# zichunhao/lgn-autoencoder

Hardware: AMD Instinct MI355X
Metric: jets/sec fwd+bwd, 30-particle maxdim=2 bs=512 (higher is better)
Workload: dtype f64

## Files before the change

### lgn-autoencoder_amd/csrc/api.hip

```cpp
#include "net.hpp"

using namespace lgn;

extern "C" {

int lgn_level_fwd_f64(int B, int N, int C, int CO, int decoder, const double* s_in, const double* v_in, const double* p,
                      const uint8_t* mask, const double* ra, const double* rb, const double* rc, const double* w0,
                      const double* b0, const double* w1, const double* b1, const double* wm0, const double* wm1,
                      double* ag0, double* ag1, double* s_out, double* v_out, void* stream) {
  LGN_CHECK_ARG(s_in && v_in && p && b0 && b1 && wm0 && wm1 && ag0 && ag1 && s_out && v_out, "level_fwd: null pointer");
  LGN_CHECK_ARG(decoder || (mask && ra && rb && rc && w0 && w1), "level_fwd: encoder needs mask and radial parameters");
  LevelArgs<double> a{B, N, C, CO, s_in, v_in, p, mask, ra, rb, rc, w0, b0, w1, b1, wm0, wm1, ag0, ag1, s_out, v_out};
  a.flags = level_flags_from_env();
  return level_fwd_dispatch<double>(a, decoder, (hipStream_t)stream);
}

int lgn_level_bwd_partial_rows(int B, int N, int decoder, int* rows_mix, int* rows_rad) {
  LGN_CHECK_ARG(B > 0 && N > 0 && rows_mix && rows_rad, "level_bwd_partial_rows: bad arguments");
  level_bwd_partial_rows(B, N, decoder, level_flags_from_env(), rows_mix, rows_rad);
  return 0;
}

int lgn_level_rad_partial_len(int C, int decoder) { return rad_partial_size(C, decoder != 0); }
int lgn_level_jet_split(int B, int N) { return N <= 40 ? level_jet_split(B, N) : 1; }

int lgn_level_bwd_f64(int B, int N, int C, int CO, int decoder, const double* s_in, const double* v_in, const double* p,
                      const uint8_t* mask, const double* ra, const double* rb, const double* rc, const double* w0,
                      const double* b0, const double* w1, const double* b1, const double* wm0, const double* wm1,
                      const double* ag0, const double* ag1, const double* g_s_out, const double* g_v_out, double* g_ag,
                      double* g_s_in, double* g_v_in, double* g_p, double* part_mix, double* part_rad, void* stream) {
  LGN_CHECK_ARG(s_in && v_in && p && b0 && b1 && wm0 && wm1 && ag0 && ag1 && g_s_out && g_v_out && g_ag && g_s_in &&
                    g_v_in && part_mix && part_rad, "level_bwd: null pointer");
  LGN_CHECK_ARG(decoder ? (g_p != nullptr) : (mask && ra && rb && rc && w0 && w1), "level_bwd: missing decoder g_p / encoder radial parameters");
  LevelBwdArgs<double> a{B, N, C, CO, s_in, v_in, p, mask, ra, rb, rc, w0, b0, w1, b1, wm0, wm1, ag0, ag1,
                         g_s_out, g_v_out, g_ag, g_s_in, g_v_in, g_p, part_mix, part_rad};
  a.flags = level_flags_from_env();
  return level_bwd_dispatch<double>(a, decoder, (hipStream_t)stream);
}

int lgn_cg_product_fwd_f64(int R, int N, int C, int D1, int D2, int DO, int mode, int nnz, const int* row_ptr, const int* col,
                           const double* coef, const double* x1, const double* x2, double* out, void* stream) {
  return cg_product_fwd(R, N, C, D1, D2, DO, mode, nnz, row_ptr, col, coef, x1, x2, out, (hipStream_t)stream);
}
int lgn_cg_product_bwd_f64(int R, int N, int C, int D1, int D2, int DO, int mode, int nnz, const int* row_ptr, const int* col,
                           const double* coef, const double* x1, const double* x2, const double* g_out, double* g_x1, double* g_x2,
                           void* stream) {
  return cg_product_bwd(R, N, C, D1, D2, DO, mode, nnz, row_ptr, col, coef, x1, x2, g_out, g_x1, g_x2, (hipStream_t)stream);
}

int lgn_reduce_partials_f64(const double* part, int rows, int n, double* out, int accumulate, void* stream) {
  LGN_CHECK_ARG(part && out && rows > 0 && n >= 0, "reduce_partials: bad arguments");
// ... 172 lines not shown
```

### lgn-autoencoder_amd/csrc/level_bwd.hip

```cpp
#include <stdlib.h>

#include "level_dev.hpp"
#include <type_traits>
#include "ops.hpp"
#include "tail_dev.hpp"

namespace lgn {

template <int C> struct GA {
  static constexpr int A3 = 0, A4 = 2 * C, A1 = 4 * C, A2 = 12 * C, SIZE = 20 * C;
};

template <typename T, int C>
__global__ __launch_bounds__(BLOCK) void level_bwd_mix_kernel(LevelBwdArgs<T> a) {
  constexpr int IT = 32;
  constexpr int K = 5 * C;
  constexpr int XS = K * 10;
  const int N = a.N, B = a.B, CO = a.CO;
  const int b = blockIdx.x, tile = blockIdx.y, tid = threadIdx.x;
  const int GS = CO * 10;

  extern __shared__ __align__(16) unsigned char smem_raw[];
  T* sm = reinterpret_cast<T*>(smem_raw);
  T* wm = sm;
// ... 338 lines not shown
    }
  }
  return 0;
}

int level_bwd_nodes2_dispatch(const LevelBwdArgs<double>& a, int decoder, hipStream_t stream);
int level_bwd_rad2_dispatch(const LevelBwdArgs<double>& a, hipStream_t stream);

int level_bwd3_dispatch(const LevelBwdArgs<double>& a, int decoder, hipStream_t stream);
int level_bwd_dec_sep_dispatch(const LevelBwdArgs<double>& a, hipStream_t stream);
int level_bwd_sweep_enc_dispatch(const LevelBwdArgs<double>& a, hipStream_t stream);
static bool dec_pairwise(int flags) { return (flags & LVL_DEC_PAIRWISE) != 0; }
bool level_bwd3_fits(int N);

static bool use_v3(int N, int flags) { return !(flags & LVL_LEVEL_V2) && level_bwd3_fits(N); }

bool level_bwd_carries_input(int N, int flags) { return use_v3(N, flags); }

void level_bwd_partial_rows(int B, int N, int decoder, int flags, int* rows_mix, int* rows_rad) {
  const int tiles = cdiv(N, 32);
  if (use_v3(N, flags)) {
    const int split = (decoder && !dec_pairwise(flags)) ? 1 : level_jet_split(B, N);
    *rows_mix = B * split;
    *rows_rad = B * split;
    return;
  }
  *rows_mix = B * tiles;
  if (decoder && dec_pairwise(flags)) {
    *rows_rad = B * tiles;
  } else {
// ... 135 lines not shown
```

### lgn-autoencoder_amd/csrc/level_bwd3.hip

```cpp
#include "level_dev.hpp"
#include "ops.hpp"
#include "wave_sum.hpp"

namespace lgn {

typedef double v4d __attribute__((ext_vector_type(4)));

namespace {
__device__ __forceinline__ double dppq(double v, int xor2) {
  int lo = __double2loint(v), hi = __double2hiint(v);
  if (xor2) {
    lo = __builtin_amdgcn_mov_dpp(lo, 0x4E, 0xF, 0xF, true);
    hi = __builtin_amdgcn_mov_dpp(hi, 0x4E, 0xF, 0xF, true);
  } else {
    lo = __builtin_amdgcn_mov_dpp(lo, 0xB1, 0xF, 0xF, true);
    hi = __builtin_amdgcn_mov_dpp(hi, 0xB1, 0xF, 0xF, true);
  }
  return __hiloint2double(hi, lo);
}
__device__ __forceinline__ double quad_sum(double v) {
  v += dppq(v, 0);
  v += dppq(v, 1);
  return v;
}
// ... 34 lines not shown
  static constexpr int SMS = 52;
  static constexpr int SEPSZ = DEC ? SMS * C : 0;
  static size_t smem(int N, int CO) {
    return sizeof(double) * ((((size_t)N * NS + 1) & ~size_t(1)) + (size_t)N * (20 * C + 2) + (size_t)N * 10 * C + (size_t)N * PS +
                             scratch(N, CO) + SEPSZ) + N + 16;
  }
};

template <int C, bool DEC, bool SEP, int NWV, bool SYM = false>
__global__ __launch_bounds__(64 * NWV) __attribute__((amdgpu_waves_per_eu(C <= 4 || DEC ? 2 : 1, C <= 4 || DEC ? 2 : 1))) void level_bwd3_kernel(LevelBwdArgs<double> a) {
  static_assert(!SYM || !DEC, "the symmetric sweep is the encoder's");
  using F = Bwd3<C, DEC, NWV>;
  constexpr int BLK = F::BLK;
  using G = GA3<C>;
  constexpr int NG = F::NG, NS = F::NS, PS = F::PS, K = 5 * C;
  const int N = a.N, B = a.B, CO = a.CO;
  const int b = blockIdx.x, tid = threadIdx.x, lane = tid & 63, wave = tid >> 6;
  const int ngroups = (N + 3) >> 2, gper = (ngroups + (int)gridDim.y - 1) / (int)gridDim.y;
  const int glo = min(ngroups, (int)blockIdx.y * gper), ghi = min(ngroups, glo + gper);
  const int nlo = min(N, 4 * glo), nhi = min(N, 4 * ghi);
  const size_t prow = (size_t)b * gridDim.y + blockIdx.y;

  extern __shared__ __align__(16) unsigned char smem_raw[];
  double* nd = reinterpret_cast<double*>(smem_raw);
  double* ga = nd + ((N * NS + 1) & ~1);
  double* gd = ga + N * G::SIZE;
  double* pj = gd + N * 10 * C;
  double* tr = pj + N * PS;
  double* go = tr;
  double* wm = go + N * 10 * CO;
  double* agl = wm + 4 * CO * K;
  double* sm = tr + F::scratch(N, CO);
  uint8_t* mk = reinterpret_cast<uint8_t*>(sm + F::SEPSZ);

  STAMP(0);
  {
    const size_t plo = (size_t)B * N * CO, pa = (size_t)B * N * 2 * C;
    JetRegs<double> jr;
    load_jet_issue<double, C, DEC>(a.s_in, a.v_in, a.p, a.mask, B, N, b, jr);
    const int eg = tid < N * CO ? tid : 0, ea_ = tid < N * 2 * C ? tid : 0, ew = tid < 2 * CO * K ? tid : 0;
    const size_t ig = (size_t)b * N * CO + eg, ia = (size_t)b * N * 2 * C + ea_;
    double rg[10], ra[10];
    rg[0] = a.g_s_out[ig];
    rg[1] = a.g_s_out[plo + ig];
    ra[0] = a.ag0[ia];
    ra[1] = a.ag0[pa + ia];
#pragma unroll
    for (int m = 0; m < 4; ++m) {
      rg[2 + m] = a.g_v_out[ig * 4 + m];
      rg[6 + m] = a.g_v_out[plo * 4 + ig * 4 + m];
      ra[2 + m] = a.ag1[ia * 4 + m];
      ra[6 + m] = a.ag1[(pa + ia) * 4 + m];
    }
    const double w0v = a.wm0[ew], w1v = a.wm1[ew];
    load_jet_commit<double, C, DEC>(a.s_in, a.v_in, a.p, a.mask, B, N, b, jr, nd, pj, mk);
    if (tid < N * CO) {
#pragma unroll
      for (int m = 0; m < 10; ++m) go[tid * 10 + m] = rg[m];
    }
    if (tid < N * 2 * C) {
#pragma unroll
      for (int m = 0; m < 10; ++m) agl[tid * 10 + m] = ra[m];
    }
    if (tid < 2 * CO * K) {
      wm[tid] = w0v;
      wm[2 * CO * K + tid] = w1v;
    }
    for (int e = tid + BLK; e < 2 * CO * K; e += BLK) {
      wm[e] = a.wm0[e];
      wm[2 * CO * K + e] = a.wm1[e];
    }
    for (int e = tid + BLK; e < N * CO; e += BLK) {
      const size_t idx = (size_t)b * N * CO + e;
      double* g = go + e * 10;
      g[0] = a.g_s_out[idx];
      g[1] = a.g_s_out[plo + idx];
#pragma unroll
      for (int m = 0; m < 4; ++m) {
        g[2 + m] = a.g_v_out[idx * 4 + m];
        g[6 + m] = a.g_v_out[plo * 4 + idx * 4 + m];
      }
    }
    for (int e = tid + BLK; e < N * 2 * C; e += BLK) {
      const size_t ea = (size_t)b * N * 2 * C + e;
      double* x = agl + e * 10;
      x[0] = a.ag0[ea];
      x[1] = a.ag0[pa + ea];
#pragma unroll
      for (int m = 0; m < 4; ++m) {
        x[2 + m] = a.ag1[ea * 4 + m];
        x[6 + m] = a.ag1[(pa + ea) * 4 + m];
      }
    }
  }
  __syncthreads();
  STAMP(1);

  {
    const int half = tid >= BLK / 2;
    for (int e = half ? tid - BLK / 2 : tid; e < N * C; e += BLK / 2) {
      const int n = e / C, c = e - n * C;
      const double* w0r = wm + c;
      const double* w1r = wm + 2 * CO * K + c;
      if (half == 0) {
        cx<double> gx0[2] = {{0, 0}, {0, 0}}, gx1[2][4] = {{{0, 0}, {0, 0}, {0, 0}, {0, 0}}, {{0, 0}, {0, 0}, {0, 0}, {0, 0}}};
        for (int o = 0; o < CO; ++o) {
          const double* g = go + (n * CO + o) * 10;
          const cx<double> gs = {g[0], g[1]};
          cx<double> gv[4];
#pragma unroll
          for (int m = 0; m < 4; ++m) gv[m] = {g[2 + m], g[6 + m]};
// ... 48 lines not shown
#pragma unroll
        for (int m = 0; m < 4; ++m) {
          cfmac(gs, b34[m], v[m]);
          cx<double> gv = b2[m];
          cfmac(gv, b34[m], s);
          cfmac(gv, a3, vt[m]);
          gdn[2 + m] = gv.r;
          gdn[6 + m] = gv.i;
        }
        gdn[0] = gs.r;
        gdn[1] = gs.i;
      }
    }
  }
  STAMP(2);
  {
    double* part = a.part_mix + prow * (4 * CO * K);
    constexpr int NPART = F::MIXP;
    const int OK = CO * K, nper = (nhi - nlo + NPART - 1) / NPART;
    const int pi = tid / K, k = tid - pi * K;
    cx<double> d0[8], d1[8];
#pragma unroll
    for (int o = 0; o < 8; ++o) d0[o] = d1[o] = {0, 0};
    if (pi < NPART) {
      const int q = k / C, c = k - q * C;
      const int n1 = min(nhi, nlo + (pi + 1) * nper);
      for (int n = nlo + pi * nper; n < n1; ++n) {
        cx<double> x0, x1[4];
        if (q < 2) {
          const double* x = agl + (n * 2 * C + k) * 10;
          x0 = {x[0], x[1]};
#pragma unroll
          for (int m = 0; m < 4; ++m) x1[m] = {x[2 + m], x[6 + m]};
        } else {
          const double* ni = nd + n * NS + c * 10;
          const cx<double> s = {ni[0], ni[1]};
          cx<double> v[4];
#pragma unroll
          for (int m = 0; m < 4; ++m) v[m] = {ni[2 + m], ni[6 + m]};
          if (q == 2) {
            x0 = s;
#pragma unroll
            for (int m = 0; m < 4; ++m) x1[m] = v[m];
          } else {
            if (q == 3) { x0 = bil2(v, v); x0.r *= 0.5; x0.i *= 0.5; } else x0 = cmul(s, s);
#pragma unroll
            for (int m = 0; m < 4; ++m) x1[m] = cmul(v[m], s);
          }
// ... 22 lines not shown
    }
    STAMP(50);
    __syncthreads();
    STAMP(51);
    for (int ex = tid; ex < 4 * OK; ex += BLK) {
      const int e = ex >> 2, x = ex & 3;
      double v = red[ex];
#pragma unroll
      for (int pp = 1; pp < NPART; ++pp) v += red[pp * OK * 4 + ex];
      part[x * OK + e] = v;
    }
  }

  if constexpr (DEC && SEP) {
    STAMP(3);
    __syncthreads();
    STAMP(4);
    if (tid < 64) {
      const int k = tid & 7, part = tid >> 3;
      double mean = 0.0;
      for (int n = part; n < N; n += 8) mean += pj[n * 8 + k];
      mean += shfl_xor(mean, 8);
      mean += shfl_xor(mean, 16);
      mean += shfl_xor(mean, 32);
      if (part == 0) sm[k] = mean / N;
    }
    __syncthreads();
    for (int e = tid; e < N * 8; e += BLK) pj[e] -= sm[e & 7];
    __syncthreads();
#define LGN_PUT(k, val)                                       \
  do {                                                        \
    if ((k) < 16) a0[(k) < 16 ? (k) : 0] += (val);                                        \
    else if ((k) < 32) a1[(k) >= 16 && (k) < 32 ? (k) - 16 : 0] += (val);                 \
    else if ((k) < 44) a2[(k) >= 32 && (k) < 44 ? (k) - 32 : 0] += (val);                 \
    else a3[(k) >= 44 ? (k) - 44 : 0] += (val);                                           \
  } while (0)
    for (int c = wave; c < C; c += NWV) {
      double a0[16], a1[16], a2[12], a3[8];
#pragma unroll
      for (int k = 0; k < 16; ++k) a0[k] = a1[k] = 0.0;
#pragma unroll
      for (int k = 0; k < 12; ++k) a2[k] = 0.0;
#pragma unroll
      for (int k = 0; k < 8; ++k) a3[k] = 0.0;
      for (int n = lane; n < N; n += 64) {
        const double* ni = nd + n * NS + c * 10;
        const double* pn = pj + n * 8;
        const double* gi = ga + n * G::SIZE;
        cx<double> pc[4], v[4];
#pragma unroll
        for (int m = 0; m < 4; ++m) {
          pc[m] = {pn[m], pn[4 + m]};
          v[m] = {ni[2 + m], ni[6 + m]};
        }
        const cx<double> sn = {ni[0], ni[1]};
        LGN_PUT(0, sn.r);  LGN_PUT(1, sn.i);
#pragma unroll
        for (int m = 0; m < 4; ++m) {
          LGN_PUT(2 + 2 * m, v[m].r);  LGN_PUT(3 + 2 * m, v[m].i);
          const cx<double> sp = cmul(sn, pc[m]);
          LGN_PUT(10 + 2 * m, sp.r);  LGN_PUT(11 + 2 * m, sp.i);
        }
        const cx<double> vp = bil2(v, pc);
        LGN_PUT(18, vp.r);  LGN_PUT(19, vp.i);
        const cx<double> g3 = {0.5 * gi[G::A3 + 2 * c], 0.5 * gi[G::A3 + 2 * c + 1]};
        LGN_PUT(20, gi[G::A4 + 2 * c]);  LGN_PUT(21, gi[G::A4 + 2 * c + 1]);
        LGN_PUT(22, g3.r);  LGN_PUT(23, g3.i);
        cx<double> gp2 = {0, 0};
#pragma unroll
        for (int m = 0; m < 4; ++m) {
          const cx<double> g1 = {gi[G::A1 + (c * 4 + m) * 2], gi[G::A1 + (c * 4 + m) * 2 + 1]};
          const cx<double> g2 = {gi[G::A2 + (c * 4 + m) * 2], gi[G::A2 + (c * 4 + m) * 2 + 1]};
          LGN_PUT(24 + 2 * m, g1.r);  LGN_PUT(25 + 2 * m, g1.i);
          LGN_PUT(32 + 2 * m, g2.r);  LGN_PUT(33 + 2 * m, g2.i);
          cfmac(gp2, g2, pc[m]);
          const cx<double> gp3 = cmulc(g3, pc[m]);
          LGN_PUT(42 + 2 * m, gp3.r);  LGN_PUT(43 + 2 * m, gp3.i);
        }
        LGN_PUT(40, gp2.r);  LGN_PUT(41, gp2.i);
      }
      double* q = sm + c * F::SMS;
      wave_sum_store<16>(a0, q, lane);
      wave_sum_store<16>(a1, q + 16, lane);
      wave_sum_store<12>(a2, q + 32, lane);
      wave_sum_store<8>(a3, q + 44, lane);
    }
#undef LGN_PUT
    __syncthreads();

    STAMP(5);
    const size_t pls = (size_t)B * N * C;
    for (int e = tid; e < N * C; e += BLK) {
      const int n = e / C, c = e - n * C;
      const double* q = sm + c * F::SMS;
      const double* pn = pj + n * 8;
      const double* gdn = gd + e * 10;
      const cx<double> R0 = {a.b0[c], a.b0[c]}, R1 = {a.b1[c], a.b1[c]};
      const cx<double> e0 = {R0.r - R0.i, R0.r + R0.i};
      cx<double> pc[4], pt[4];
#pragma unroll
// ... 633 lines not shown
```

### lgn-autoencoder_amd/csrc/level_dev.hpp

```cpp
#pragma once
#include "level.hpp"

namespace lgn {

template <int C, bool DEC>
struct Carve {
  static constexpr int R = 4 * C;
  static constexpr int NS = node_stride(C);
  static constexpr int PS = DEC ? 8 : 4;
  static constexpr int RA = 0, RB = NB, RC = 2 * NB;
  static constexpr int RW = 3 * NB;
  static constexpr int RBIAS = RW + NB * R;
  static constexpr int RAD_SIZE = RBIAS + R;
  __host__ __device__ static constexpr int even(int x) { return (x + 1) & ~1; }
};

template <typename T>
struct JetRegs {
  T s[2], v[8], p[2];
  uint8_t m;
};
template <typename T, int C, bool DEC>
__device__ __forceinline__ void load_jet_issue(const T* __restrict__ s_in, const T* __restrict__ v_in, const T* __restrict__ p,
                                               const uint8_t* __restrict__ mask, int B, int N, int b, JetRegs<T>& r) {
// ... 160 lines not shown
  cx<T> t = cmul(a[2], b[2]);
  r.r -= t.r;
  r.i -= t.i;
  cfma(r, a[3], b[1]);
  return r;
}

template <typename T>
__device__ __forceinline__ void metric_perm(const cx<T> (&x)[4], cx<T> (&y)[4]) {
  y[0] = x[0];
  y[1] = x[3];
  y[2] = {-x[2].r, -x[2].i};
  y[3] = x[1];
}

__device__ __forceinline__ void rcp5(const double (&u)[5], double (&r)[5]) {
  const double p1 = u[0] * u[1], p2 = p1 * u[2], p3 = p2 * u[3], p4 = p3 * u[4];
  if (__builtin_expect(!(p4 < 0x1p+1000), 0)) {
#pragma unroll
    for (int s = 0; s < 5; ++s) r[s] = 1.0 / u[s];
    return;
  }
  double t = __builtin_amdgcn_rcp(p4);
  double e = __builtin_fma(-p4, t, 1.0);
  t = __builtin_fma(t, e, t);
  e = __builtin_fma(-p4, t, 1.0);
  t = __builtin_fma(t, e, t);
  r[4] = t * p3;  t *= u[4];
  r[3] = t * p2;  t *= u[3];
  r[2] = t * p1;  t *= u[2];
// ... 6 lines not shown
```

### lgn-autoencoder_amd/csrc/level_fwd2.hip

```cpp
#include "level_dev.hpp"
#include "net_dev.hpp"
#include "ops.hpp"
#include "wave_sum.hpp"

namespace lgn {

typedef double v4d __attribute__((ext_vector_type(4)));
LGN_STAMP_DECL
LGN_STAMP_READER(lgn_debug_stamps_fwd2)

__device__ __forceinline__ double dpp_quad(double v, int ctrl_is_xor2) {
  int lo = __double2loint(v), hi = __double2hiint(v);
  if (ctrl_is_xor2) {
    lo = __builtin_amdgcn_mov_dpp(lo, 0x4E, 0xF, 0xF, true);
    hi = __builtin_amdgcn_mov_dpp(hi, 0x4E, 0xF, 0xF, true);
  } else {
    lo = __builtin_amdgcn_mov_dpp(lo, 0xB1, 0xF, 0xF, true);
    hi = __builtin_amdgcn_mov_dpp(hi, 0xB1, 0xF, 0xF, true);
  }
  return __hiloint2double(hi, lo);
}
__device__ __forceinline__ double quad_sum(double v) {
  v += dpp_quad(v, 0);
  v += dpp_quad(v, 1);
// ... 118 lines not shown
    }
  }
#pragma unroll
  for (int g = 0; g < NG; ++g) {
    const int ch = 4 * g + cg;
#pragma unroll
    for (int q = 0; q < 4; ++q) {
      const double* bb = (q >> 1) ? a.b1 : a.b0;
      bias[g][q] = ch < C ? (DEC ? bb[ch] : bb[2 * ch + (q & 1)]) : 0.0;
    }
  }
  __syncthreads();
  STAMP(1);

  if constexpr (DEC && SEP) {
    if (tid < 64) {
      const int k = tid & 7, part = tid >> 3;
      double mean = 0.0;
      for (int n = part; n < N; n += 8) mean += pj[n * 8 + k];
      mean += shfl_xor(mean, 8);
      mean += shfl_xor(mean, 16);
      mean += shfl_xor(mean, 32);
      if (part == 0) sums[k] = mean / N;
    }
    __syncthreads();
    for (int e = tid; e < N * 8; e += nthr) pj[e] -= sums[e & 7];
    __syncthreads();
#define LGN_PUT(k, val)                                           \
  do {                                                            \
    if ((k) < 12) a0[(k) < 12 ? (k) : 0] += (val);                \
    else a1[(k) >= 12 ? (k) - 12 : 0] += (val);                   \
  } while (0)
    for (int c = wave; c < C; c += nw) {
      double a0[12], a1[8];
#pragma unroll
      for (int k = 0; k < 12; ++k) a0[k] = 0.0;
#pragma unroll
      for (int k = 0; k < 8; ++k) a1[k] = 0.0;
      for (int n = lane; n < N; n += 64) {
        const double* ni = nd + n * F::NS + c * 10;
        const double* pn = pj + n * 8;
        const cx<double> sn = {ni[0], ni[1]};
        cx<double> v[4], pc[4];
#pragma unroll
        for (int m = 0; m < 4; ++m) {
          v[m] = {ni[2 + m], ni[6 + m]};
          pc[m] = {pn[m], pn[4 + m]};
        }
        LGN_PUT(0, sn.r);  LGN_PUT(1, sn.i);
#pragma unroll
        for (int m = 0; m < 4; ++m) {
          LGN_PUT(2 + 2 * m, v[m].r);  LGN_PUT(3 + 2 * m, v[m].i);
          const cx<double> sp = cmul(sn, pc[m]);
          LGN_PUT(10 + 2 * m, sp.r);  LGN_PUT(11 + 2 * m, sp.i);
        }
        const cx<double> vp = bil2(v, pc);
        LGN_PUT(18, vp.r);  LGN_PUT(19, vp.i);
      }
      wave_sum_store<12>(a0, sums + c * 20, lane);
      wave_sum_store<8>(a1, sums + c * 20 + 12, lane);
    }
#undef LGN_PUT
    __syncthreads();
  }

  const int ngroups = (N + 3) >> 2, gper = (ngroups + (int)gridDim.y - 1) / (int)gridDim.y;
  const int rlo = min(N, 4 * (int)blockIdx.y * gper), rhi = min(N, rlo + 4 * gper);
  auto catmix = [&](int c0, int c1) {
    constexpr int K = 5 * C;
    const int nr = c1 - c0;
    const size_t plo = (size_t)B * N * CO;
    if (wave == 0) {
      for (int rl = lane; rl < nr; rl += 64) {
        const int r = c0 + rl;
        const double* st = agl + rl * F::AGS;
        const double* ni = nd + r * F::NS;
        cx<double> x[K];
// ... 45 lines not shown
          cx<double> acc = {0, 0};
#pragma unroll
          for (int k = 0; k < K; ++k) cfma(acc, cx<double>{wr[k], wi[k]}, x[k]);
          const size_t e = ((size_t)b * N + r) * CO + o;
          a.v_out[e * 4 + m] = acc.r;
          a.v_out[plo * 4 + e * 4 + m] = acc.i;
        }
      }
    }
    };
  for (int c0 = rlo; c0 < rhi; c0 += chunk) {
  const int c1 = min(rhi, c0 + chunk);
  if constexpr (DEC && SEP) {
    for (int e = tid; e < (c1 - c0) * C; e += nthr) {
      const int rl = e / C, c = e - rl * C, n = c0 + rl;
      const double* sm = sums + c * 20;
      const double* pn = pj + n * 8;
      const cx<double> R0 = {a.b0[c], a.b0[c]}, R1 = {a.b1[c], a.b1[c]};
      const cx<double> e0 = {R0.r - R0.i, R0.r + R0.i};
      const cx<double> S = {sm[0], sm[1]};
      cx<double> VS[4], pc[4];
#pragma unroll
      for (int m = 0; m < 4; ++m) {
        VS[m] = {sm[2 + 2 * m], sm[3 + 2 * m]};
        pc[m] = {pn[m], pn[4 + m]};
      }
      double* st = agl + rl * F::AGS;
      const cx<double> a4 = cmul(S, e0);
      cx<double> t = bil2(VS, pc);
      t.r -= sm[18];  t.i -= sm[19];
      cx<double> a3 = cmul(R1, t);
      st[F::A3 + 2 * c] = 0.5 * a3.r;  st[F::A3 + 2 * c + 1] = 0.5 * a3.i;
      st[F::A4 + 2 * c] = a4.r;        st[F::A4 + 2 * c + 1] = a4.i;
#pragma unroll
      for (int m = 0; m < 4; ++m) {
        const cx<double> a1 = cmul(VS[m], e0);
        cx<double> u = cmul(pc[m], S);
        u.r -= sm[10 + 2 * m];  u.i -= sm[11 + 2 * m];
        const cx<double> a2 = cmul(R1, u);
        st[F::A1 + (c * 4 + m) * 2] = a1.r;  st[F::A1 + (c * 4 + m) * 2 + 1] = a1.i;
        st[F::A2 + (c * 4 + m) * 2] = a2.r;  st[F::A2 + (c * 4 + m) * 2 + 1] = a2.i;
      }
    }
  } else {
  const int ngr = (c1 - c0 + 3) >> 2;
  const int rs = (!DEC && nw == 4 && ngr >= 1 && ngr <= 2 && chunk >= 16) ? 4 / ngr : 1;
  const int rpart = rs > 1 ? wave % rs : 0, ntl = (N + 3) >> 2;
  auto row_group = [&](const int rg, const int jlo, const int jhi, const int slab) __attribute__((always_inline)) {
    const int i0 = rg * 4;
    const int i = i0 + ti;
    const bool iok = i < N;
    const int ii = iok ? i : N - 1;
    double pi[F::PS];
#pragma unroll
    for (int m = 0; m < F::PS; ++m) pi[m] = pj[ii * F::PS + m];
    const bool mi = DEC ? false : (mk[ii] != 0);
// ... 147 lines not shown
    for (int rg = (c0 >> 2) + wave; rg * 4 < c1; rg += nw) row_group(rg, 0, N, 0);
  }
  if (rs > 1) {
    __syncthreads();
    const int tot = 4 * ngr * F::AGS;
    for (int e = tid; e < tot; e += nthr) {
      double v = agl[e];
      for (int pp = 1; pp < rs; ++pp) v += agl[pp * tot + e];
      agl[e] = v;
    }
  }
  }
  __syncthreads();
  STAMP(20);

  if constexpr (TRAIN) {
    const size_t pl0 = (size_t)B * N * 2 * C;
    for (int e = tid; e < (c1 - c0) * 2 * C; e += nthr) {
      const int n = e / (2 * C), r = e - n * 2 * C, blk = r / C, ch = r - blk * C;
      const double* st = agl + n * F::AGS + (blk ? F::A4 : F::A3) + 2 * ch;
      const size_t ge = ((size_t)b * N + c0) * 2 * C + e;
      a.ag0[ge] = st[0];
      a.ag0[pl0 + ge] = st[1];
    }
    for (int e = tid; e < (c1 - c0) * 2 * C * 4; e += nthr) {
      const int n = e / (8 * C), r = e - n * 8 * C, blk = r / (4 * C), cm = r - blk * 4 * C;
      const double* st = agl + n * F::AGS + (blk ? F::A2 : F::A1) + 2 * cm;
      const size_t ge = ((size_t)b * N + c0) * 8 * C + e;
      a.ag1[ge] = st[0];
      a.ag1[pl0 * 4 + ge] = st[1];
    }
// ... 38 lines not shown
  auto kern = level_fwd2_kernel<C, DEC, SEP, TRAIN>;
  if (smem > 64 * 1024) {
    hipError_t e = hipFuncSetAttribute(reinterpret_cast<const void*>(kern), hipFuncAttributeMaxDynamicSharedMemorySize, (int)smem);
    if (e != hipSuccess) { set_error("hipFuncSetAttribute: %s", hipGetErrorString(e)); return (int)e; }
  }
  const int nthreads = wide ? 2 * BLOCK : BLOCK;
  const int split = (SEP || a.N > 40) ? 1 : level_jet_split(a.B, a.N);
  hipLaunchKernelGGL(kern, dim3(a.B, split), dim3(nthreads), smem, stream, a, chunk);
  LGN_CHECK_LAUNCH();
  return 0;
}

bool level_fwd_carries_loss(int N, int flags) { return N <= 40 && !(flags & LVL_DEC_PAIRWISE); }

template <bool TRAIN>
static int level_fwd_run(const LevelArgs<double>& a, int decoder, hipStream_t stream) {
  LGN_CHECK_ARG(a.B > 0 && a.N > 0, "level_fwd: empty batch (B=%d N=%d)", a.B, a.N);
  LGN_CHECK_ARG(!a.in_w0 || (!decoder && a.in_w1 && a.in_s && a.in_v), "level_fwd: the input stage rides on encoder levels only");
  LGN_CHECK_ARG(a.CO >= 1 && a.CO <= 8, "level_fwd: C_out=%d unsupported (1..8)", a.CO);
  const bool pairwise = (a.flags & LVL_DEC_PAIRWISE) != 0;
#define LGN_CASE(CC)                                                                                         \
  case CC:                                                                                                   \
    if (!decoder) return launch_level_fwd2<CC, false, false, TRAIN>(a, stream);                              \
    return pairwise ? launch_level_fwd2<CC, true, false, TRAIN>(a, stream) : launch_level_fwd2<CC, true, true, TRAIN>(a, stream);
  switch (a.C) {
#ifdef LGN_DEV_ONLY_C4
    LGN_CASE(4)
#else
    LGN_CASE(1) LGN_CASE(2) LGN_CASE(3) LGN_CASE(4) LGN_CASE(5) LGN_CASE(6) LGN_CASE(7) LGN_CASE(8)
#endif
    default:
// ... 15 lines not shown
```

### lgn-autoencoder_amd/csrc/ops.hpp

```cpp
#pragma once
#include <cstdlib>
#include <vector>
#include "level.hpp"

namespace lgn {

template <typename T> int level_fwd_dispatch(const LevelArgs<T>&, int decoder, hipStream_t);
int level_fwd_eval(const LevelArgs<double>&, int decoder, hipStream_t);
template <typename T> int level_bwd_dispatch(const LevelBwdArgs<T>&, int decoder, hipStream_t);
template <typename T> int reduce_partials(const T* part, int rows, int n, T* out, int accumulate, hipStream_t);
template <typename T> int reduce_partials_strided(const T* part, int rows, int stride, int col0, int n, T* out, hipStream_t);
constexpr int RED_MAX_SEG = 64;
template <typename T> struct RedSeg { const T* part; int rows, stride, col0, n; T* out; };
template <typename T> struct RedJob {
  int nseg;
  RedSeg<T> seg[RED_MAX_SEG];
  int tile0[RED_MAX_SEG + 1];
  void add(const T* part, int rows, int stride, int col0, int n, T* out) { seg[nseg++] = RedSeg<T>{part, rows, stride, col0, n, out}; }
};
template <typename T> int reduce_segments(RedJob<T>& job, hipStream_t);
template <typename T>
int rad_finalize(const T* tot, int C, const T* ra, const T* rb, const T* rc, const T* w0, const T* w1, T* g_a, T* g_b, T* g_c,
                 T* g_w0, T* g_b0, T* g_w1, T* g_b1, hipStream_t);
struct RadFinJob {
// ... 7 lines not shown
  double *m, *v;
  long* step_dev;
  double lambda, lr, beta1, beta2, eps;
  int do_adam;
  const double* loss_part;
  int nB;
  double* loss_out;
  int reduce_only;
  unsigned long long* counters;
  int opt_form = 0;
  int kind = 0;
  double l2 = 0.0, alpha = 0.0, mu = 0.0;
};
int step_tail(const std::vector<RedSeg<double>>& segs, const RadFinJob& fin, const StepTailArgs& ta, hipStream_t st);
void level_bwd_partial_rows(int B, int N, int decoder, int flags, int* rows_mix, int* rows_rad);
bool level_bwd_carries_input(int N, int flags);
bool level_fwd_carries_loss(int N, int flags);

constexpr int MLP_MAX_LIN = 8;
template <typename T>
struct MlpArgs {
  int M;
  int C;
  int H;
  int nlin;
  const T* w[MLP_MAX_LIN];
  const T* b[MLP_MAX_LIN];
  const T* s_in;
  T* s_out;
  const T* g_out;
// ... 127 lines not shown
```

### lgn-autoencoder_amd/csrc/step.hip

```cpp
#include <stdlib.h>

#include <algorithm>
#include <mutex>
#include <vector>

#include "net.hpp"
#include "../../include/lgn_amd.h"

namespace lgn {
namespace {

struct Bump {
  double* base;
  size_t off = 0;
  double* take(size_t n) {
    n = (n + 15) & ~size_t(15);
    double* p = base ? base + off : nullptr;
    off += n;
    return p;
  }
};

struct NetBuf {
  double *s[5], *v[5], *smix[4], *ag0[4], *ag1[4];
// ... 139 lines not shown
  Work w{};
  Bump b{base};
  const int Nd = dec_nodes(d), Nmax = d.N > Nd ? d.N : Nd;
  const size_t BNe = (size_t)d.B * d.N, BNd = (size_t)d.B * Nd, BN = (size_t)d.B * Nmax;
  const int L = d.n_levels;
  int cmax = 0;
  for (int l = 0; l <= L; ++l) cmax = cmax > d.enc_channels[l] ? cmax : d.enc_channels[l], cmax = cmax > d.dec_channels[l] ? cmax : d.dec_channels[l];
  auto net = [&](NetBuf& n, const int* ch, bool dec) {
    const size_t BN = dec ? BNd : BNe;
    for (int l = 0; l <= L; ++l) {
      n.s[l] = b.take(2 * BN * ch[l]);
      n.v[l] = b.take(8 * BN * ch[l]);
    }
    for (int l = 0; l < L; ++l) {
      n.smix[l] = b.take(2 * BN * ch[l + 1]);
      n.ag0[l] = b.take(4 * BN * ch[l]);
      n.ag1[l] = b.take(16 * BN * ch[l]);
      const size_t hs = l + 1 < L && BN <= mlp_save_max_rows()
                            ? mlp_saved_doubles((int)BN, d.mlp_hidden_mul * 2 * ch[l + 1], d.mlp_nlin) : 0;
      n.hsave[l] = hs ? b.take(hs) : nullptr;
    }
  };
  net(w.enc, d.enc_channels, false);
  net(w.dec, d.dec_channels, true);
  const int Ts = d.tau_s, Tv = d.tau_v, PB = pool_blocks(d.latent_pool);
  w.lat_s = b.take((size_t)2 * d.B * PB * Ts);
  w.lat_v = b.take((size_t)2 * d.B * PB * Tv * 4);
  w.g_lat_v = b.take((size_t)2 * d.B * PB * Tv * 4);
  w.pdec = b.take(8 * BN);
  for (int q = 0; q < 2; ++q) {
    w.gs[q] = b.take(2 * BN * cmax);
    w.gv[q] = b.take(8 * BN * cmax);
// ... 708 lines not shown
  double* pdec;
  int* idx;
  size_t total;
};
NetAct carve_act(const lgn_net_desc& d, bool dec, double* base) {
  NetAct a{};
  Bump b{base};
  const size_t BN = (size_t)d.B * d.N;
  const int* ch = dec ? d.dec_channels : d.enc_channels;
  for (int l = 0; l <= d.n_levels; ++l) {
    a.n.s[l] = b.take(2 * BN * ch[l]);
    a.n.v[l] = b.take(8 * BN * ch[l]);
  }
  for (int l = 0; l < d.n_levels; ++l) {
    a.n.smix[l] = b.take(2 * BN * ch[l + 1]);
    a.n.ag0[l] = b.take(4 * BN * ch[l]);
    a.n.ag1[l] = b.take(16 * BN * ch[l]);
    const size_t hs = BN <= mlp_save_max_rows()
                          ? mlp_saved_doubles((int)BN, d.mlp_hidden_mul * 2 * ch[l + 1], d.mlp_nlin) : 0;
    a.n.hsave[l] = hs ? b.take(hs) : nullptr;
  }
  if (dec) a.pdec = b.take(8 * BN);
  else a.idx = reinterpret_cast<int*>(b.take(((size_t)d.B * 2 * (d.tau_s + d.tau_v) * 2 + 1) / 2 + 8));
  a.total = b.off;
  return a;
}

struct NetScratch {
  Work w;
  size_t total;
};
NetScratch carve_scratch(const lgn_net_desc& d, bool dec, double* base) {
// ... 591 lines not shown
```

Measured before the change: 1.067 million.

## Recompute decoder separable aggregates in backward instead of storing them

For the decoder's separable (non-pairwise) path under the v3 backward, the forward no longer writes the per-node aggregate tensors ag0/ag1, and no workspace is allocated for them. The backward kernel instead rebuilds them: it recentres the momenta, computes per-channel jet sums into shared memory, and evaluates the aggregate on the fly in the mix-gradient loop. The shared helper code is factored out of the forward kernel. This removes global writes and reads of the aggregates and shrinks the workspace, at the cost of extra arithmetic, an extra barrier and shared-memory reductions in the backward.

```diff
diff --git a/lgn-autoencoder_amd/csrc/api.hip b/lgn-autoencoder_amd/csrc/api.hip
--- a/lgn-autoencoder_amd/csrc/api.hip
+++ b/lgn-autoencoder_amd/csrc/api.hip
@@ -8,10 +8,12 @@
                       const uint8_t* mask, const double* ra, const double* rb, const double* rc, const double* w0,
                       const double* b0, const double* w1, const double* b1, const double* wm0, const double* wm1,
                       double* ag0, double* ag1, double* s_out, double* v_out, void* stream) {
-  LGN_CHECK_ARG(s_in && v_in && p && b0 && b1 && wm0 && wm1 && ag0 && ag1 && s_out && v_out, "level_fwd: null pointer");
+  const int flags = level_flags_from_env();
+  LGN_CHECK_ARG(s_in && v_in && p && b0 && b1 && wm0 && wm1 && s_out && v_out && ((ag0 && ag1) || !level_saves_aggregate(N, decoder, flags)),
+                "level_fwd: null pointer");
   LGN_CHECK_ARG(decoder || (mask && ra && rb && rc && w0 && w1), "level_fwd: encoder needs mask and radial parameters");
   LevelArgs<double> a{B, N, C, CO, s_in, v_in, p, mask, ra, rb, rc, w0, b0, w1, b1, wm0, wm1, ag0, ag1, s_out, v_out};
-  a.flags = level_flags_from_env();
+  a.flags = flags;
   return level_fwd_dispatch<double>(a, decoder, (hipStream_t)stream);
 }
 
@@ -29,12 +31,13 @@
                       const double* b0, const double* w1, const double* b1, const double* wm0, const double* wm1,
                       const double* ag0, const double* ag1, const double* g_s_out, const double* g_v_out, double* g_ag,
                       double* g_s_in, double* g_v_in, double* g_p, double* part_mix, double* part_rad, void* stream) {
-  LGN_CHECK_ARG(s_in && v_in && p && b0 && b1 && wm0 && wm1 && ag0 && ag1 && g_s_out && g_v_out && g_ag && g_s_in &&
-                    g_v_in && part_mix && part_rad, "level_bwd: null pointer");
+  const int flags = level_flags_from_env();
+  LGN_CHECK_ARG(s_in && v_in && p && b0 && b1 && wm0 && wm1 && g_s_out && g_v_out && g_ag && g_s_in && g_v_in && part_mix && part_rad &&
+                    ((ag0 && ag1) || !level_saves_aggregate(N, decoder, flags)), "level_bwd: null pointer");
   LGN_CHECK_ARG(decoder ? (g_p != nullptr) : (mask && ra && rb && rc && w0 && w1), "level_bwd: missing decoder g_p / encoder radial parameters");
   LevelBwdArgs<double> a{B, N, C, CO, s_in, v_in, p, mask, ra, rb, rc, w0, b0, w1, b1, wm0, wm1, ag0, ag1,
                          g_s_out, g_v_out, g_ag, g_s_in, g_v_in, g_p, part_mix, part_rad};
-  a.flags = level_flags_from_env();
+  a.flags = flags;
   return level_bwd_dispatch<double>(a, decoder, (hipStream_t)stream);
 }
 
diff --git a/lgn-autoencoder_amd/csrc/level_bwd.hip b/lgn-autoencoder_amd/csrc/level_bwd.hip
--- a/lgn-autoencoder_amd/csrc/level_bwd.hip
+++ b/lgn-autoencoder_amd/csrc/level_bwd.hip
@@ -376,6 +376,8 @@
 bool level_bwd3_fits(int N);
 
 static bool use_v3(int N, int flags) { return !(flags & LVL_LEVEL_V2) && level_bwd3_fits(N); }
+
+bool level_saves_aggregate(int N, int decoder, int flags) { return !(decoder && !dec_pairwise(flags) && use_v3(N, flags)); }
 
 bool level_bwd_carries_input(int N, int flags) { return use_v3(N, flags); }
 
diff --git a/lgn-autoencoder_amd/csrc/level_bwd3.hip b/lgn-autoencoder_amd/csrc/level_bwd3.hip
--- a/lgn-autoencoder_amd/csrc/level_bwd3.hip
+++ b/lgn-autoencoder_amd/csrc/level_bwd3.hip
@@ -72,6 +72,7 @@
   constexpr int BLK = F::BLK;
   using G = GA3<C>;
   constexpr int NG = F::NG, NS = F::NS, PS = F::PS, K = 5 * C;
+  constexpr bool REBUILD = DEC && SEP;
   const int N = a.N, B = a.B, CO = a.CO;
   const int b = blockIdx.x, tid = threadIdx.x, lane = tid & 63, wave = tid >> 6;
   const int ngroups = (N + 3) >> 2, gper = (ngroups + (int)gridDim.y - 1) / (int)gridDim.y;
@@ -101,14 +102,19 @@
     double rg[10], ra[10];
     rg[0] = a.g_s_out[ig];
     rg[1] = a.g_s_out[plo + ig];
-    ra[0] = a.ag0[ia];
-    ra[1] = a.ag0[pa + ia];
 #pragma unroll
     for (int m = 0; m < 4; ++m) {
       rg[2 + m] = a.g_v_out[ig * 4 + m];
       rg[6 + m] = a.g_v_out[plo * 4 + ig * 4 + m];
-      ra[2 + m] = a.ag1[ia * 4 + m];
-      ra[6 + m] = a.ag1[(pa + ia) * 4 + m];
+    }
+    if constexpr (!REBUILD) {
+      ra[0] = a.ag0[ia];
+      ra[1] = a.ag0[pa + ia];
+#pragma unroll
+      for (int m = 0; m < 4; ++m) {
+        ra[2 + m] = a.ag1[ia * 4 + m];
+        ra[6 + m] = a.ag1[(pa + ia) * 4 + m];
+      }
     }
     const double w0v = a.wm0[ew], w1v = a.wm1[ew];
     load_jet_commit<double, C, DEC>(a.s_in, a.v_in, a.p, a.mask, B, N, b, jr, nd, pj, mk);
@@ -116,9 +122,11 @@
 #pragma unroll
       for (int m = 0; m < 10; ++m) go[tid * 10 + m] = rg[m];
     }
-    if (tid < N * 2 * C) {
-#pragma unroll
-      for (int m = 0; m < 10; ++m) agl[tid * 10 + m] = ra[m];
+    if constexpr (!REBUILD) {
+      if (tid < N * 2 * C) {
+#pragma unroll
+        for (int m = 0; m < 10; ++m) agl[tid * 10 + m] = ra[m];
+      }
     }
     if (tid < 2 * CO * K) {
       wm[tid] = w0v;
@@ -139,20 +147,26 @@
         g[6 + m] = a.g_v_out[plo * 4 + idx * 4 + m];
       }
     }
-    for (int e = tid + BLK; e < N * 2 * C; e += BLK) {
-      const size_t ea = (size_t)b * N * 2 * C + e;
-      double* x = agl + e * 10;
-      x[0] = a.ag0[ea];
-      x[1] = a.ag0[pa + ea];
-#pragma unroll
-      for (int m = 0; m < 4; ++m) {
-        x[2 + m] = a.ag1[ea * 4 + m];
-        x[6 + m] = a.ag1[(pa + ea) * 4 + m];
+    if constexpr (!REBUILD) {
+      for (int e = tid + BLK; e < N * 2 * C; e += BLK) {
+        const size_t ea = (size_t)b * N * 2 * C + e;
+        double* x = agl + e * 10;
+        x[0] = a.ag0[ea];
+        x[1] = a.ag0[pa + ea];
+#pragma unroll
+        for (int m = 0; m < 4; ++m) {
+          x[2 + m] = a.ag1[ea * 4 + m];
+          x[6 + m] = a.ag1[(pa + ea) * 4 + m];
+        }
       }
     }
   }
   __syncthreads();
   STAMP(1);
+  if constexpr (REBUILD) {
+    sep_centre_momenta(pj, N, sm);
+    for (int c = wave; c < C; c += NWV) sep_jet_sums<NS>(nd, pj, N, c, lane, sm + c * F::SMS);
+  }
 
   {
     const int half = tid >= BLK / 2;
@@ -231,6 +245,7 @@
     }
   }
   STAMP(2);
+  if constexpr (REBUILD) __syncthreads();
   {
     double* part = a.part_mix + prow * (4 * CO * K);
     constexpr int NPART = F::MIXP;
@@ -242,13 +257,23 @@
     if (pi < NPART) {
       const int q = k / C, c = k - q * C;
       const int n1 = min(nhi, nlo + (pi + 1) * nper);
+      double b0c = 0.0, b1c = 0.0;
+      if constexpr (REBUILD) { b0c = a.b0[c]; b1c = a.b1[c]; }
       for (int n = nlo + pi * nper; n < n1; ++n) {
         cx<double> x0, x1[4];
         if (q < 2) {
-          const double* x = agl + (n * 2 * C + k) * 10;
-          x0 = {x[0], x[1]};
-#pragma unroll
-          for (int m = 0; m < 4; ++m) x1[m] = {x[2 + m], x[6 + m]};
+          if constexpr (REBUILD) {
+            cx<double> a3, a4, a1[4], a2[4];
+            sep_aggregate(sm + c * F::SMS, pj + n * 8, b0c, b1c, a3, a4, a1, a2);
+            x0 = q == 0 ? a3 : a4;
+#pragma unroll
+            for (int m = 0; m < 4; ++m) x1[m] = q == 0 ? a1[m] : a2[m];
+          } else {
+            const double* x = agl + (n * 2 * C + k) * 10;
+            x0 = {x[0], x[1]};
+#pragma unroll
+            for (int m = 0; m < 4; ++m) x1[m] = {x[2 + m], x[6 + m]};
+          }
         } else {
           const double* ni = nd + n * NS + c * 10;
           const cx<double> s = {ni[0], ni[1]};
@@ -301,55 +326,22 @@
 
   if constexpr (DEC && SEP) {
     STAMP(3);
-    __syncthreads();
     STAMP(4);
-    if (tid < 64) {
-      const int k = tid & 7, part = tid >> 3;
-      double mean = 0.0;
-      for (int n = part; n < N; n += 8) mean += pj[n * 8 + k];
-      mean += shfl_xor(mean, 8);
-      mean += shfl_xor(mean, 16);
-      mean += shfl_xor(mean, 32);
-      if (part == 0) sm[k] = mean / N;
-    }
-    __syncthreads();
-    for (int e = tid; e < N * 8; e += BLK) pj[e] -= sm[e & 7];
-    __syncthreads();
 #define LGN_PUT(k, val)                                       \
   do {                                                        \
-    if ((k) < 16) a0[(k) < 16 ? (k) : 0] += (val);                                        \
-    else if ((k) < 32) a1[(k) >= 16 && (k) < 32 ? (k) - 16 : 0] += (val);                 \
-    else if ((k) < 44) a2[(k) >= 32 && (k) < 44 ? (k) - 32 : 0] += (val);                 \
-    else a3[(k) >= 44 ? (k) - 44 : 0] += (val);                                           \
+    if ((k) < 36) a1[(k) >= 20 && (k) < 36 ? (k) - 20 : 0] += (val);                      \
+    else a2[(k) >= 36 ? (k) - 36 : 0] += (val);                                           \
   } while (0)
     for (int c = wave; c < C; c += NWV) {
-      double a0[16], a1[16], a2[12], a3[8];
-#pragma unroll
-      for (int k = 0; k < 16; ++k) a0[k] = a1[k] = 0.0;
-#pragma unroll
-      for (int k = 0; k < 12; ++k) a2[k] = 0.0;
-#pragma unroll
-      for (int k = 0; k < 8; ++k) a3[k] = 0.0;
+      double a1[16], a2[16];
+#pragma unroll
+      for (int k = 0; k < 16; ++k) a1[k] = a2[k] = 0.0;
       for (int n = lane; n < N; n += 64) {
-        const double* ni = nd + n * NS + c * 10;
         const double* pn = pj + n * 8;
         const double* gi = ga + n * G::SIZE;
-        cx<double> pc[4], v[4];
-#pragma unroll
-        for (int m = 0; m < 4; ++m) {
-          pc[m] = {pn[m], pn[4 + m]};
-          v[m] = {ni[2 + m], ni[6 + m]};
-        }
-        const cx<double> sn = {ni[0], ni[1]};
-        LGN_PUT(0, sn.r);  LGN_PUT(1, sn.i);
-#pragma unroll
-        for (int m = 0; m < 4; ++m) {
-          LGN_PUT(2 + 2 * m, v[m].r);  LGN_PUT(3 + 2 * m, v[m].i);
-          const cx<double> sp = cmul(sn, pc[m]);
-          LGN_PUT(10 + 2 * m, sp.r);  LGN_PUT(11 + 2 * m, sp.i);
-        }
-        const cx<double> vp = bil2(v, pc);
-        LGN_PUT(18, vp.r);  LGN_PUT(19, vp.i);
+        cx<double> pc[4];
+#pragma unroll
+        for (int m = 0; m < 4; ++m) pc[m] = {pn[m], pn[4 + m]};
         const cx<double> g3 = {0.5 * gi[G::A3 + 2 * c], 0.5 * gi[G::A3 + 2 * c + 1]};
         LGN_PUT(20, gi[G::A4 + 2 * c]);  LGN_PUT(21, gi[G::A4 + 2 * c + 1]);
         LGN_PUT(22, g3.r);  LGN_PUT(23, g3.i);
@@ -367,10 +359,8 @@
         LGN_PUT(40, gp2.r);  LGN_PUT(41, gp2.i);
       }
       double* q = sm + c * F::SMS;
-      wave_sum_store<16>(a0, q, lane);
-      wave_sum_store<16>(a1, q + 16, lane);
-      wave_sum_store<12>(a2, q + 32, lane);
-      wave_sum_store<8>(a3, q + 44, lane);
+      wave_sum_store<16>(a1, q + 20, lane);
+      wave_sum_store<16>(a2, q + 36, lane);
     }
 #undef LGN_PUT
     __syncthreads();
diff --git a/lgn-autoencoder_amd/csrc/level_dev.hpp b/lgn-autoencoder_amd/csrc/level_dev.hpp
--- a/lgn-autoencoder_amd/csrc/level_dev.hpp
+++ b/lgn-autoencoder_amd/csrc/level_dev.hpp
@@ -1,5 +1,6 @@
 #pragma once
 #include "level.hpp"
+#include "wave_sum.hpp"
 
 namespace lgn {
 
@@ -198,6 +199,84 @@
   y[3] = x[1];
 }
 
+__device__ __forceinline__ void sep_centre_momenta(double* pj, int N, double* mean8) {
+  const int tid = threadIdx.x, nthr = blockDim.x;
+  if (tid < 64) {
+    const int k = tid & 7, part = tid >> 3;
+    double mean = 0.0;
+    for (int n = part; n < N; n += 8) mean += pj[n * 8 + k];
+    mean += shfl_xor(mean, 8);
+    mean += shfl_xor(mean, 16);
+    mean += shfl_xor(mean, 32);
+    if (part == 0) mean8[k] = mean / N;
+  }
+  __syncthreads();
+  for (int e = tid; e < N * 8; e += nthr) pj[e] -= mean8[e & 7];
+  __syncthreads();
+}
+
+template <int NS>
+__device__ __forceinline__ void sep_jet_sums(const double* nd, const double* pj, int N, int c, int lane, double* dst) {
+#define LGN_PUT(k, val)                                           \
+  do {                                                            \
+    if ((k) < 12) a0[(k) < 12 ? (k) : 0] += (val);                \
+    else a1[(k) >= 12 ? (k) - 12 : 0] += (val);                   \
+  } while (0)
+  double a0[12], a1[8];
+#pragma unroll
+  for (int k = 0; k < 12; ++k) a0[k] = 0.0;
+#pragma unroll
+  for (int k = 0; k < 8; ++k) a1[k] = 0.0;
+  for (int n = lane; n < N; n += 64) {
+    const double* ni = nd + n * NS + c * 10;
+    const double* pn = pj + n * 8;
+    const cx<double> sn = {ni[0], ni[1]};
+    cx<double> v[4], pc[4];
+#pragma unroll
+    for (int m = 0; m < 4; ++m) {
+      v[m] = {ni[2 + m], ni[6 + m]};
+      pc[m] = {pn[m], pn[4 + m]};
+    }
+    LGN_PUT(0, sn.r);  LGN_PUT(1, sn.i);
+#pragma unroll
+    for (int m = 0; m < 4; ++m) {
+      LGN_PUT(2 + 2 * m, v[m].r);  LGN_PUT(3 + 2 * m, v[m].i);
+      const cx<double> sp = cmul(sn, pc[m]);
+      LGN_PUT(10 + 2 * m, sp.r);  LGN_PUT(11 + 2 * m, sp.i);
+    }
+    const cx<double> vp = bil2(v, pc);
+    LGN_PUT(18, vp.r);  LGN_PUT(19, vp.i);
+  }
+  wave_sum_store<12>(a0, dst, lane);
+  wave_sum_store<8>(a1, dst + 12, lane);
+#undef LGN_PUT
+}
+
+__device__ __forceinline__ void sep_aggregate(const double* sm, const double* pn, double b0c, double b1c, cx<double>& a3,
+                                              cx<double>& a4, cx<double> (&a1)[4], cx<double> (&a2)[4]) {
+  const cx<double> R0 = {b0c, b0c}, R1 = {b1c, b1c};
+  const cx<double> e0 = {R0.r - R0.i, R0.r + R0.i};
+  const cx<double> S = {sm[0], sm[1]};
+  cx<double> VS[4], pc[4];
+#pragma unroll
+  for (int m = 0; m < 4; ++m) {
+    VS[m] = {sm[2 + 2 * m], sm[3 + 2 * m]};
+    pc[m] = {pn[m], pn[4 + m]};
+  }
+  a4 = cmul(S, e0);
+  cx<double> t = bil2(VS, pc);
+  t.r -= sm[18];  t.i -= sm[19];
+  const cx<double> r3 = cmul(R1, t);
+  a3 = {0.5 * r3.r, 0.5 * r3.i};
+#pragma unroll
+  for (int m = 0; m < 4; ++m) {
+    a1[m] = cmul(VS[m], e0);
+    cx<double> u = cmul(pc[m], S);
+    u.r -= sm[10 + 2 * m];  u.i -= sm[11 + 2 * m];
+    a2[m] = cmul(R1, u);
+  }
+}
+
 __device__ __forceinline__ void rcp5(const double (&u)[5], double (&r)[5]) {
   const double p1 = u[0] * u[1], p2 = p1 * u[2], p3 = p2 * u[3], p4 = p3 * u[4];
   if (__builtin_expect(!(p4 < 0x1p+1000), 0)) {
diff --git a/lgn-autoencoder_amd/csrc/level_fwd2.hip b/lgn-autoencoder_amd/csrc/level_fwd2.hip
--- a/lgn-autoencoder_amd/csrc/level_fwd2.hip
+++ b/lgn-autoencoder_amd/csrc/level_fwd2.hip
@@ -156,53 +156,8 @@
   STAMP(1);
 
   if constexpr (DEC && SEP) {
-    if (tid < 64) {
-      const int k = tid & 7, part = tid >> 3;
-      double mean = 0.0;
-      for (int n = part; n < N; n += 8) mean += pj[n * 8 + k];
-      mean += shfl_xor(mean, 8);
-      mean += shfl_xor(mean, 16);
-      mean += shfl_xor(mean, 32);
-      if (part == 0) sums[k] = mean / N;
-    }
-    __syncthreads();
-    for (int e = tid; e < N * 8; e += nthr) pj[e] -= sums[e & 7];
-    __syncthreads();
-#define LGN_PUT(k, val)                                           \
-  do {                                                            \
-    if ((k) < 12) a0[(k) < 12 ? (k) : 0] += (val);                \
-    else a1[(k) >= 12 ? (k) - 12 : 0] += (val);                   \
-  } while (0)
-    for (int c = wave; c < C; c += nw) {
-      double a0[12], a1[8];
-#pragma unroll
-      for (int k = 0; k < 12; ++k) a0[k] = 0.0;
-#pragma unroll
-      for (int k = 0; k < 8; ++k) a1[k] = 0.0;
-      for (int n = lane; n < N; n += 64) {
-        const double* ni = nd + n * F::NS + c * 10;
-        const double* pn = pj + n * 8;
-        const cx<double> sn = {ni[0], ni[1]};
-        cx<double> v[4], pc[4];
-#pragma unroll
-        for (int m = 0; m < 4; ++m) {
-          v[m] = {ni[2 + m], ni[6 + m]};
-          pc[m] = {pn[m], pn[4 + m]};
-        }
-        LGN_PUT(0, sn.r);  LGN_PUT(1, sn.i);
-#pragma unroll
-        for (int m = 0; m < 4; ++m) {
-          LGN_PUT(2 + 2 * m, v[m].r);  LGN_PUT(3 + 2 * m, v[m].i);
-          const cx<double> sp = cmul(sn, pc[m]);
-          LGN_PUT(10 + 2 * m, sp.r);  LGN_PUT(11 + 2 * m, sp.i);
-        }
-        const cx<double> vp = bil2(v, pc);
-        LGN_PUT(18, vp.r);  LGN_PUT(19, vp.i);
-      }
-      wave_sum_store<12>(a0, sums + c * 20, lane);
-      wave_sum_store<8>(a1, sums + c * 20 + 12, lane);
-    }
-#undef LGN_PUT
+    sep_centre_momenta(pj, N, sums);
+    for (int c = wave; c < C; c += nw) sep_jet_sums<F::NS>(nd, pj, N, c, lane, sums + c * 20);
     __syncthreads();
   }
 
@@ -278,32 +233,15 @@
   if constexpr (DEC && SEP) {
     for (int e = tid; e < (c1 - c0) * C; e += nthr) {
       const int rl = e / C, c = e - rl * C, n = c0 + rl;
-      const double* sm = sums + c * 20;
-      const double* pn = pj + n * 8;
-      const cx<double> R0 = {a.b0[c], a.b0[c]}, R1 = {a.b1[c], a.b1[c]};
-      const cx<double> e0 = {R0.r - R0.i, R0.r + R0.i};
-      const cx<double> S = {sm[0], sm[1]};
-      cx<double> VS[4], pc[4];
+      cx<double> a3, a4, a1[4], a2[4];
+      sep_aggregate(sums + c * 20, pj + n * 8, a.b0[c], a.b1[c], a3, a4, a1, a2);
+      double* st = agl + rl * F::AGS;
+      st[F::A3 + 2 * c] = a3.r;  st[F::A3 + 2 * c + 1] = a3.i;
+      st[F::A4 + 2 * c] = a4.r;  st[F::A4 + 2 * c + 1] = a4.i;
 #pragma unroll
       for (int m = 0; m < 4; ++m) {
-        VS[m] = {sm[2 + 2 * m], sm[3 + 2 * m]};
-        pc[m] = {pn[m], pn[4 + m]};
-      }
-      double* st = agl + rl * F::AGS;
-      const cx<double> a4 = cmul(S, e0);
-      cx<double> t = bil2(VS, pc);
-      t.r -= sm[18];  t.i -= sm[19];
-      cx<double> a3 = cmul(R1, t);
-      st[F::A3 + 2 * c] = 0.5 * a3.r;  st[F::A3 + 2 * c + 1] = 0.5 * a3.i;
-      st[F::A4 + 2 * c] = a4.r;        st[F::A4 + 2 * c + 1] = a4.i;
-#pragma unroll
-      for (int m = 0; m < 4; ++m) {
-        const cx<double> a1 = cmul(VS[m], e0);
-        cx<double> u = cmul(pc[m], S);
-        u.r -= sm[10 + 2 * m];  u.i -= sm[11 + 2 * m];
-        const cx<double> a2 = cmul(R1, u);
-        st[F::A1 + (c * 4 + m) * 2] = a1.r;  st[F::A1 + (c * 4 + m) * 2 + 1] = a1.i;
-        st[F::A2 + (c * 4 + m) * 2] = a2.r;  st[F::A2 + (c * 4 + m) * 2 + 1] = a2.i;
+        st[F::A1 + (c * 4 + m) * 2] = a1[m].r;  st[F::A1 + (c * 4 + m) * 2 + 1] = a1[m].i;
+        st[F::A2 + (c * 4 + m) * 2] = a2[m].r;  st[F::A2 + (c * 4 + m) * 2 + 1] = a2[m].i;
       }
     }
   } else {
@@ -481,7 +419,7 @@
   __syncthreads();
   STAMP(20);
 
-  if constexpr (TRAIN) {
+  if (TRAIN && (!(DEC && SEP) || a.ag0 != nullptr)) {
     const size_t pl0 = (size_t)B * N * 2 * C;
     for (int e = tid; e < (c1 - c0) * 2 * C; e += nthr) {
       const int n = e / (2 * C), r = e - n * 2 * C, blk = r / C, ch = r - blk * C;
@@ -550,7 +488,11 @@
 bool level_fwd_carries_loss(int N, int flags) { return N <= 40 && !(flags & LVL_DEC_PAIRWISE); }
 
 template <bool TRAIN>
-static int level_fwd_run(const LevelArgs<double>& a, int decoder, hipStream_t stream) {
+static int level_fwd_run(const LevelArgs<double>& args, int decoder, hipStream_t stream) {
+  const bool keep = TRAIN && level_saves_aggregate(args.N, decoder, args.flags);
+  LGN_CHECK_ARG(!keep || (args.ag0 && args.ag1), "level_fwd: no buffer for the aggregate the backward reads");
+  LevelArgs<double> a = args;
+  if (!keep) a.ag0 = a.ag1 = nullptr;
   LGN_CHECK_ARG(a.B > 0 && a.N > 0, "level_fwd: empty batch (B=%d N=%d)", a.B, a.N);
   LGN_CHECK_ARG(!a.in_w0 || (!decoder && a.in_w1 && a.in_s && a.in_v), "level_fwd: the input stage rides on encoder levels only");
   LGN_CHECK_ARG(a.CO >= 1 && a.CO <= 8, "level_fwd: C_out=%d unsupported (1..8)", a.CO);
diff --git a/lgn-autoencoder_amd/csrc/ops.hpp b/lgn-autoencoder_amd/csrc/ops.hpp
--- a/lgn-autoencoder_amd/csrc/ops.hpp
+++ b/lgn-autoencoder_amd/csrc/ops.hpp
@@ -45,6 +45,7 @@
 };
 int step_tail(const std::vector<RedSeg<double>>& segs, const RadFinJob& fin, const StepTailArgs& ta, hipStream_t st);
 void level_bwd_partial_rows(int B, int N, int decoder, int flags, int* rows_mix, int* rows_rad);
+bool level_saves_aggregate(int N, int decoder, int flags);
 bool level_bwd_carries_input(int N, int flags);
 bool level_fwd_carries_loss(int N, int flags);
 
diff --git a/lgn-autoencoder_amd/csrc/step.hip b/lgn-autoencoder_amd/csrc/step.hip
--- a/lgn-autoencoder_amd/csrc/step.hip
+++ b/lgn-autoencoder_amd/csrc/step.hip
@@ -177,8 +177,9 @@
     }
     for (int l = 0; l < L; ++l) {
       n.smix[l] = b.take(2 * BN * ch[l + 1]);
-      n.ag0[l] = b.take(4 * BN * ch[l]);
-      n.ag1[l] = b.take(16 * BN * ch[l]);
+      const bool keep = level_saves_aggregate(dec ? Nd : d.N, dec, d.flags);
+      n.ag0[l] = keep ? b.take(4 * BN * ch[l]) : nullptr;
+      n.ag1[l] = keep ? b.take(16 * BN * ch[l]) : nullptr;
       const size_t hs = l + 1 < L && BN <= mlp_save_max_rows()
                             ? mlp_saved_doubles((int)BN, d.mlp_hidden_mul * 2 * ch[l + 1], d.mlp_nlin) : 0;
       n.hsave[l] = hs ? b.take(hs) : nullptr;
@@ -917,8 +918,9 @@
   }
   for (int l = 0; l < d.n_levels; ++l) {
     a.n.smix[l] = b.take(2 * BN * ch[l + 1]);
-    a.n.ag0[l] = b.take(4 * BN * ch[l]);
-    a.n.ag1[l] = b.take(16 * BN * ch[l]);
+    const bool keep = level_saves_aggregate(d.N, dec, d.flags);
+    a.n.ag0[l] = keep ? b.take(4 * BN * ch[l]) : nullptr;
+    a.n.ag1[l] = keep ? b.take(16 * BN * ch[l]) : nullptr;
     const size_t hs = BN <= mlp_save_max_rows()
                           ? mlp_saved_doubles((int)BN, d.mlp_hidden_mul * 2 * ch[l + 1], d.mlp_nlin) : 0;
     a.n.hsave[l] = hs ? b.take(hs) : nullptr;
```

Result: no change. 1.075 million, median of 6 (+0.8%).
